# jay-tux/cutrace

Measured on AMD Instinct MI355X. Metric: Mrays/sec (primary+secondary), higher is better.
Workload: dtype f32; 1 GPU; bunny.json@1920x1080 bounces=5 fudge=1e-3, 1 frame(s)/step row-tiled over 1 GPU(s), gather to rank 0; steps_in_flight=1

## Files before the change

cutrace_amd/__init__.py:

```python
import contextlib
import ctypes as C
import os

import numpy as np

from . import _lib
from ._lib import Camera, Light, Material, Object, RenderStats, Rows, SceneDesc, Triangle, Vec3

ROOT = _lib.ROOT

VAR_AUTO = 0
VAR_NO_PREFILTER = 2
VAR_NO_ANYHIT = 4
VAR_NO_CLUSTER = 8
VAR_STATS = 16
VAR_EXACT_POW = 32
VAR_NO_REORDER = 256
VAR_NO_OCC6 = 512
VAR_NO_DIRECT = 1024
VAR_IMAGE_ORDER_FIRST = 2048
VAR_MERGE = 4096
VAR_IGNORE_TRANSPARENT = 8192

RAY_IGNORE_TRANSPARENT = 1
# ... 395 lines not shown
        shape = C.c_uint32()
        _check("ctr_debug_last_shape", _lib.hip_lib().ctr_debug_last_shape(self._h, C.byref(shape)))
        return int(shape.value)

    def last_opaque(self):
        opaque = C.c_uint32()
        _check("ctr_debug_last_opaque", _lib.hip_lib().ctr_debug_last_opaque(self._h, C.byref(opaque)))
        return int(opaque.value)

    def room_facts(self):
        out = np.zeros(5, np.float32)
        lights = C.c_uint32()
        _check("ctr_debug_room_facts", _lib.hip_lib().ctr_debug_room_facts(self._h, out.ctypes.data, C.byref(lights)))
        return {"c": out[:3].copy(), "r": float(out[3]), "delta": float(out[4]), "lights": int(lights.value)}

    @staticmethod
    def lane_stats(reset=True):
        raw = np.zeros(96, np.uint64)
        _check("ctr_debug_lane_stats", _lib.hip_lib().ctr_debug_lane_stats(raw.ctypes.data, 1 if reset else 0))
        c = [int(x) for x in raw]
        trips, live = c[72], c[73]
        out = {"wave_trips": trips, "live_lanes_per_trip": live / trips if trips else None,
               "live_fraction": live / (64.0 * trips) if trips else None,
               "live_fraction_of_in_image_lanes": (live / trips) / (c[75] / c[74]) if trips and c[74] and c[75] else None,
               "trips_by_live_lanes_1_8_to_57_64": c[64:72], "trips_mixing_kinds": c[76], "waves": c[74],
               "merged_walks": c[78], "merged_walks_redone": c[77],
               "shadow_casts_at_meshes": {"wave_casts": c[80], "receivers_all_off_mesh": c[81], "of_those_unoccluded_by_meshes": c[82],
                                          "unoccluded_by_meshes_any_receiver": c[83]},
               "anyhit_shadow_trips": c[88], "anyhit_shadow_trips_without_planes": c[89]}
        kinds = {}
        for d in range(16):
            for name, base in (("radiance", 0), ("shadow", 16)):
                if c[32 + base + d]:
                    label = "primary" if (name == "radiance" and d == 0) else f"{name}@depth{d}"
                    kinds[label] = {"lanes": c[base + d], "trips": c[32 + base + d],
                                    "lanes_per_trip": c[base + d] / c[32 + base + d]}
        out["by_kind"] = kinds
        return out

    def _torch_device(self):
        import torch
        return torch.device("cuda", self.device)

    def _rays_arg(self, x, what, cols):
# ... 453 lines not shown
```

cutrace_amd/_lib.py:

```python
import ctypes as C
import os

PKG = os.path.dirname(os.path.abspath(__file__))
ROOT = os.path.dirname(PKG)


class Vec3(C.Structure):
    _fields_ = [("x", C.c_float), ("y", C.c_float), ("z", C.c_float)]

    def tup(self):
        return (self.x, self.y, self.z)


class Triangle(C.Structure):
    _fields_ = [("p1", Vec3), ("p2", Vec3), ("p3", Vec3)]


class Object(C.Structure):
    _fields_ = [("type", C.c_uint32), ("reserved", C.c_uint32), ("mat_idx", C.c_uint64),
                ("v0", Vec3), ("v1", Vec3), ("v2", Vec3), ("f0", C.c_float),
                ("tri_begin", C.c_uint64), ("tri_count", C.c_uint64)]


class Light(C.Structure):
# ... 137 lines not shown
        "ctr_scene_set_cameras": ([_ptr, _P(Camera), _u32], _int),
        "ctr_render_device_batch": ([_ptr, _f32, _int, _P(Rows), _u32, _u32, _u64, _u32, _ptr, _ptr, _ptr, _ptr, _ptr], _int),
        "ctr_algorithmic_bytes": ([_ptr, _f32, _int, _P(Rows), _P(_u64), _P(_u64)], _int),
        "ctr_frame_alloc": ([_u64, _P(_f32p), _P(_f32p), _P(_f32p)], _int),
        "ctr_frame_free": ([_f32p], None),
        "ctr_tile_costs": ([_ptr, _ptr, _u64, _P(_u64)], _int),
        "ctr_last_counters": ([_ptr, _ptr], _int),
        "ctr_selftest_exact_math": ([_P(_u64)], _int),
        "ctr_debug_poison_next_order": ([_ptr], _int),
        "ctr_render_uv": ([_ptr, _f32, _int, _P(Rows), _ptr, _ptr, _ptr, _ptr, _P(RenderStats)], _int),
        "ctr_debug_lane_stats": ([_ptr, _int], _int),
        "ctr_debug_last_kernel": ([_ptr, _P(_u32)], _int),
        "ctr_debug_last_shape": ([_ptr, _P(_u32)], _int),
        "ctr_debug_last_opaque": ([_ptr, _P(_u32)], _int),
        "ctr_debug_room_facts": ([_ptr, _ptr, _P(_u32)], _int),
        "ctr_multi_create": ([_P(SceneDesc), _P(_int), _int, _P(_ptr)], _int),
        "ctr_multi_destroy": ([_ptr], None),
        "ctr_multi_devices": ([_ptr], _int),
        "ctr_multi_transport": ([_ptr], _str),
        "ctr_multi_size": ([_ptr, _P(_u64), _P(_u64)], _int),
        "ctr_multi_set_size": ([_ptr, _u64, _u64], _int),
        "ctr_multi_set_variant": ([_ptr, _u32], _int),
        "ctr_render_multi": ([_ptr, _f32, _int, _u64, _ptr, _ptr, _ptr, _P(RenderStats)], _int),
        "ctr_multi_kernel_ms": ([_ptr, _P(C.c_double), _int], _int),
        "ctr_reinterleave_device": ([_P(ReintPart), _u32, _u64, _u64, _u64, _ptr, _ptr, _ptr, _ptr], _int),
        "ctr_multi_submit": ([_ptr, _f32, _int, _u64, _ptr, _ptr, _ptr], _int),
        "ctr_multi_wait": ([_ptr, _P(RenderStats)], _int),
    },
    "cutrace_rays.h": {
        "ctr_cast_rays": ([_ptr, _P(RayQuery), _ptr], _int),
# ... 103 lines not shown
```

cutrace_amd/csrc/ctr_internal.h:

```cpp
#ifndef CUTRACE_AMD_CTR_INTERNAL_H
#define CUTRACE_AMD_CTR_INTERNAL_H

#include <hip/hip_runtime_api.h>
#include <string.h>

#include <memory>
#include <mutex>
#include <string>
#include <utility>
#include <vector>

#include "cutrace_amd.h"
#include "guard_scan.h"
#include "lbvh.h"
#include "mesh_refit.h"
#include "scene_device.h"
#include "scene_flatten.h"
#include "tile_order_policy.h"

#pragma GCC visibility push(hidden)
int fail(int code, const std::string &msg);
int hip_fail(hipError_t e, const char *what);
#define HIP_TRY(expr)                                     \
  do {                                                    \
// ... 51 lines not shown

struct ctr_scene {
  int device = 0;
  FlatScene flat;
  SceneBuf d_objs{sizeof(DObj)}, d_oloop{sizeof(DObj)}, d_meshes{sizeof(DObj)}, d_planes{sizeof(DPlanePair)}, d_tris{sizeof(DTri)};
  SceneBuf d_nodes{sizeof(DNode)}, d_nodes4{sizeof(DNode4)}, d_gnorm{4 * sizeof(float)}, d_lights{sizeof(DLight)}, d_mats{sizeof(DMat)};
  DCam cam{};
  GrowBuf d_cams{sizeof(DCam)};
  uint32_t n_cams = 0;
  uint32_t cams_epoch = 0;
  std::vector<DCam> h_cams;
  uint32_t user_variant = CTR_VAR_AUTO;
  bool no_scene_head = false;
  bool no_shape_build = false;
  bool no_wall_skip = false;
  bool no_opaque_build = false;
  struct RoomWords { float c[3], r, delta; uint32_t lights; } last_room{};
  GrowBuf out{7 * sizeof(float)};
  GrowBuf uv{2 * sizeof(float)};
  GrowBuf img{9};
  GrowBuf d_groups{sizeof(uint32_t)};
  GrowBuf h_groups{sizeof(uint32_t), true};
  GrowBuf h_counters{sizeof(unsigned long long), true};
  unsigned long long last_cnt[16] = {0};
  GrowBuf d_counters{sizeof(unsigned long long)};
  GrowBuf d_shards{sizeof(unsigned long long)};
  uint32_t last_kernel = 0;
  uint32_t last_shape = 0;
  uint32_t last_opaque = 0;
  OrderState order;
  GrowBuf d_cost{sizeof(uint32_t)}, d_order{sizeof(uint32_t)};
  bool poison_next_order = false;
// ... 56 lines not shown
```

cutrace_amd/csrc/ctr_render.cpp:

```cpp
#include <hip/hip_runtime_api.h>

#include <chrono>
#include <cstdio>
#include <cstdlib>

#include "ctr_internal.h"
#include "cutrace_aa.h"
#include "cutrace_images.h"
#include "cutrace_lens.h"
#include "frame_images.h"
#include "kernel_choice.h"
#include "row_parts.h"
#include "tile_order.h"
#include "tile_shape.h"

#ifndef CTR_OCC6_MIN_TRIS
#define CTR_OCC6_MIN_TRIS 1000
#endif

uint64_t ctr_scene::occ6_min_tris() {
  static const uint64_t v = [] { const char *e = getenv("CUTRACE_OCC6_MIN_TRIS"); return e ? (uint64_t)atoll(e) : (uint64_t)CTR_OCC6_MIN_TRIS; }();
  return v;
}

// ... 113 lines not shown
  L.h = s->cam.h;
  L.first_frame = c.first_frame;
  L.n_frames = c.n_frames;
  L.frame_stride_px = c.frame_stride_px;
  L.fudge = c.fudge;
  L.bounces = c.bounces;
  L.ss_log2 = c.ss_log2;
}

void set_root_and_head(const ctr_scene *s, RenderLaunch &L, bool merged) {
  if (merged) L.scene.tlas_root = BVH_LEAF_FLAG | s->flat.n_mesh;
  if (!s->no_scene_head) fill_scene_head(s->flat, L.scene.tlas_root, L.head);
  L.no_shape = s->no_shape_build ? 1u : 0u;
  L.no_opaque = s->no_opaque_build ? 1u : 0u;
  if ((L.variant & KV_ANYHIT) && (ctr_launch_shape(L) == KS_ONE_MESH || (L.variant & KV_STATS))) fill_room_facts(s->flat, L.head, s->no_wall_skip);
}

ctr_scene::RoomWords room_words(const RenderLaunch &L) {
  return {{L.head.room_c[0], L.head.room_c[1], L.head.room_c[2]}, L.head.room_r, L.head.room_delta, L.head.room_lights};
}

int prepare_outputs(ctr_scene *s, RenderLaunch &L, size_t spx, const HostFrame *z) {
  if (int st = s->h_counters.reserve(16)) return st;
  if (int st = s->out.reserve(spx)) return st;
  L.depth = s->out.as<float>();
  L.color = L.depth + spx;
  L.normal = L.depth + 4 * spx;
  if (!z) return CTR_OK;
  const size_t groups = (size_t)ctr_staging_groups(L);
  if (int st = reserve_both(s->d_groups, s->h_groups, groups)) return st;
// ... 118 lines not shown
  L.variant = choice.kv;
  if (c.lens) {
    L.ray_origin = c.lens->d_origin;
    L.ray_dir = c.lens->d_dir;
    L.ray_ambient = c.lens->ambient;
  }
  if (c.ss_log2 && (st = aa_scale(L.w, L.h, L.rows, c.ss_log2, err))) return fail(st, err);
  set_root_and_head(s, L, choice.merged);
  {
    std::lock_guard<std::mutex> lk(s->mtx);
    if ((st = attach_order(s, L, big_mesh(s), false))) return st;
    s->last_kernel = L.variant;
    s->last_shape = ctr_launch_shape(L);
    s->last_opaque = ctr_launch_opaque(L);
    s->last_room = room_words(L);
  }
  return launched(ctr_launch_render(L, c.stream), "render kernel launch");
}

int render_host(ctr_scene *s, const RenderCall &c) {
  auto t0 = std::chrono::high_resolution_clock::now();
  int st = check_args(s, c.bounces);
  if (st) return st;
  std::lock_guard<std::mutex> lk(s->mtx);
  HIP_TRY(hipSetDevice(s->device));
  RenderLaunch L{};
  fill_launch(s, c, L);
  std::string err;
  if ((st = make_rows(L.h, c.rows, L.rows, err))) return fail(st, err);
  const size_t px = (size_t)L.rows.n_rows * s->cam.w;
// ... 8 lines not shown
  }
  const bool direct = choice.direct;
  const size_t spx = direct ? (size_t)ctr_staging_pixels(L) : (px ? px : 1);
  if ((st = prepare_outputs(s, L, spx, direct ? &z : nullptr))) return st;
  L.counters = s->d_counters.as<unsigned long long>();
  if (choice.reject == KR_UV_STATS) return fail(CTR_E_INVALID, "ctr_render_uv / CTR_VAR_IGNORE_TRANSPARENT: not with the counting / statistics variants");
  L.variant = s->last_kernel = choice.kv;
  if (L.variant & KV_UV) {
    if ((st = s->uv.reserve(px))) return st;
    L.uv = s->uv.as<float>();
  }
  set_root_and_head(s, L, choice.merged);
  s->last_shape = ctr_launch_shape(L);
  s->last_opaque = ctr_launch_opaque(L);
  s->last_room = room_words(L);
  if ((st = attach_order(s, L, big_mesh(s), c.count))) return st;
  HIP_TRY(hipMemsetAsync(s->d_counters.p, 0, 16 * sizeof(unsigned long long), nullptr));
  HIP_TRY(hipEventRecord(s->ev0, nullptr));
  if ((st = launched(ctr_launch_render(L, nullptr), "render kernel launch"))) return st;
  HIP_TRY(hipEventRecord(s->ev1, nullptr));
  if (px && !direct && (st = c.images ? images_out(s, L, *c.images, px) : copy_out(s, L, c.out, px))) return st;
  HIP_TRY(hipMemcpyAsync(s->h_counters.p, s->d_counters.p, 16 * sizeof(unsigned long long), hipMemcpyDeviceToHost, nullptr));
  const size_t n_groups = direct ? (size_t)ctr_staging_groups(L) : 0;
  if (direct) HIP_TRY(hipMemcpyAsync(s->h_groups.p, s->d_groups.p, n_groups * sizeof(uint32_t), hipMemcpyDeviceToHost, nullptr));
  HIP_TRY(hipStreamSynchronize(nullptr));
  if (direct && (st = check_delivery(s, L, c.out, spx, n_groups))) return st;
  return report(s, L, t0, c);
}

}
// ... 109 lines not shown
```

cutrace_amd/csrc/ctr_scene.cpp:

```cpp
#include <hip/hip_runtime_api.h>

#include <cstdio>
#include <cstdlib>
#include <cstring>
#include <mutex>
#include <string>
#include <vector>

#include "ctr_internal.h"
#include "cutrace_amd.h"
#include "guard.h"
#include "scene_device.h"
#include "scene_flatten.h"

namespace {
thread_local std::string g_err;
}

int fail(int code, const std::string &msg) {
  g_err = msg;
  fprintf(stderr, "cutrace_amd: %s\n", msg.c_str());
  return code;
}
int hip_fail(hipError_t e, const char *what) {
// ... 231 lines not shown
  int ndev = 0;
  hipError_t e = hipGetDeviceCount(&ndev);
  if (e != hipSuccess || ndev <= 0) return fail(CTR_E_NO_DEVICE, "no HIP device available (and there is no CPU fallback)");
  if (device < 0 || device >= ndev) return fail(CTR_E_INVALID, "device index out of range");
  HIP_TRY(hipSetDevice(device));
  create_stamp("device check");

  FlatScene F;
  if (int st = flatten_scene(*d, F, err)) return fail(st, err);
  auto *s = new ctr_scene();
  s->device = device;
  s->cam = to_dcam(d->cam);
  s->no_scene_head = env_switch("CUTRACE_NO_SCENE_HEAD");
  s->no_shape_build = env_switch("CUTRACE_NO_SHAPE_BUILD");
  s->no_wall_skip = env_switch("CUTRACE_NO_WALL_SKIP");
  s->no_opaque_build = env_switch("CUTRACE_NO_OPAQUE_BUILD");

  if (int st = upload_scene(s, F)) {
    ctr_scene_destroy(s);
    return hip_fail((hipError_t)(st - CTR_E_HIP_BASE), "scene upload");
  }
  create_stamp("device allocation + upload");
  s->n_cams = 1;
  s->flat = std::move(F);
  s->h_cams.assign(1, s->cam);
  create_stamp("host copies");
  if (int st = refresh_linear_meshes(s)) {
    ctr_scene_destroy(s);
    return st;
  }
// ... 99 lines not shown
  std::lock_guard<std::mutex> lk(s->mtx);
  *opaque = s->last_opaque;
  return CTR_OK;
}

int ctr_debug_room_facts(ctr_scene *s, float *out5, uint32_t *lights) {
  if (!s || !out5 || !lights) return fail(CTR_E_INVALID, "ctr_debug_room_facts: null argument");
  std::lock_guard<std::mutex> lk(s->mtx);
  for (int q = 0; q < 3; q++) out5[q] = s->last_room.c[q];
  out5[3] = s->last_room.r;
  out5[4] = s->last_room.delta;
  *lights = s->last_room.lights;
  return CTR_OK;
}

int ctr_last_counters(ctr_scene *s, uint64_t *out16) {
  if (!s || !out16) return fail(CTR_E_INVALID, "ctr_last_counters: null argument");
  std::lock_guard<std::mutex> lk(s->mtx);
  for (int q = 0; q < 16; q++) out16[q] = s->last_cnt[q];
  return CTR_OK;
}

}
```

cutrace_amd/csrc/render_kernel.hip:

```cpp
#include <hip/hip_runtime.h>
#include <math.h>
#include <stddef.h>
#include <stdint.h>
#include <stdlib.h>

#include "cutrace_amd.h"
#include "scene_device.h"
#include "bvh.h"
#include "kernel_choice.h"
#include "tile_order.h"
#include "tile_shape.h"
#include "vec3.h"

#define CADDR __attribute__((address_space(4)))
#define BALLOT(p) __builtin_amdgcn_ballot_w64(p)
#define HIDE_UNIFORM(x) asm volatile("" : "+v"(x))
#define PIN3(a, b, c) asm volatile("" : "+v"(a), "+v"(b), "+v"(c))
#define INVB(m) __builtin_amdgcn_inverse_ballot_w64(m)
#define FCMP(a, b, pred) __builtin_amdgcn_fcmpf((a), (b), (pred))
enum { FC_OEQ = 1, FC_OGT = 2, FC_OGE = 3, FC_OLT = 4, FC_OLE = 5 };
#define TL_NONE 0x7FFFFFFFu

extern "C" __device__ uint32_t ctr_writelane(uint32_t value, uint32_t lane, uint32_t old) __asm("llvm.amdgcn.writelane.i32");

// ... 104 lines not shown
  n = s;
  float y = __builtin_amdgcn_rcpf(s);
  const float e = __builtin_fmaf(-s, y, 1.0f);
  y = __builtin_fmaf(e, y, y);
  float q = y;
  const float r0 = __builtin_fmaf(-s, q, 1.0f);
  q = __builtin_fmaf(r0, y, q);
  const float r1 = __builtin_fmaf(-s, q, 1.0f);
  inv = __builtin_fmaf(r1, y, q);
}
__device__ __forceinline__ V3 vnormalized_n(V3 a, float &n) {
  float inv;
  norm_and_inverse(a.x * a.x + a.y * a.y + a.z * a.z, n, inv);
  return vscale(a, inv);
}
enum { F_R = 0, F_G, F_B, F_MAT, F_PX, F_PY, F_PZ, F_DX, F_DY, F_DZ };

struct KArgs {
  const CADDR DPlanePair *planes;
  uint32_t n_plane_recs, n_axis_recs, n_oloop, n_mesh, tlas_root, has_mesh;
  const CADDR DObj *objs;
  const CADDR float *gnorm;
  const CADDR DLight *lights;
  const CADDR DMat *mats;
  uint32_t n_light;
  int bounces;
  uint32_t n_obj, tlas_root2;
  const CADDR DObj *oloop;
  const CADDR DObj *meshes;
  uint32_t tlas_begin;
// ... 22 lines not shown

static_assert(offsetof(KArgs, planes) == 0 && offsetof(KArgs, has_mesh) == 28, "KArgs: the hot block is the first eight dwords");
static_assert(offsetof(KArgs, objs) == 32 && offsetof(KArgs, mats) == 56 && offsetof(KArgs, bounces) == 68, "KArgs: the cold block follows");

struct KParams {
  KArgs A;
  float *depth_out, *color_out, *normal_out;
  unsigned long long *counters;
};
static_assert(offsetof(KArgs, ss_log2) == 288 && offsetof(KArgs, ray_origin) == 296 && offsetof(KArgs, head) == 320, "KArgs: the lens arguments lie in the padding behind ss_log2");
static_assert(sizeof(KArgs) % 64 == 0 && offsetof(KArgs, head) % 64 == 0 && offsetof(KParams, depth_out) == sizeof(KArgs), "KParams mirrors the kernel's parameter list; the scene head lies on 64-byte lines");


constexpr uint32_t MSP_SHADOW = 0x80000000u, MSP_DONE = 0x40000000u;
constexpr uint32_t MSP_ROOM = 0x20000000u;
#define MSP_ACTIVE(m) ((int)(m) < 0x40000000)
#define MSP_IS_SHADOW(m) ((int)(m) < 0)
#define MSP_IS_RADIANCE(m) ((uint32_t)(m) < 0x40000000u)
#define MSP_DEPTH(m) ((int)((m) & 0xFFFFu))
enum { ACT_NONE = 0, ACT_LIGHT = 1, ACT_BOUNCE = 2, ACT_UNWIND = 3 };

template <uint32_t KV, uint32_t SHAPE = KS_GENERAL, bool ROOM = false, uint32_t OPQ = KO_PARENT>
__global__ __launch_bounds__(WG_THREADS, (KV & KV_OCC6) ? 6 : CTR_MIN_WAVES_EU) void render_kernel(KArgs A, float *__restrict__ depth_out,
                                                            float *__restrict__ color_out,
                                                            float *__restrict__ normal_out,
                                                            unsigned long long *__restrict__ counters) {
  constexpr bool PREFILTER = (KV & KV_PREFILTER) != 0;
  constexpr bool ANYHIT = (KV & KV_ANYHIT) != 0;
  constexpr bool COUNT = (KV & KV_COUNT) != 0;
  constexpr bool BVH = (KV & KV_BVH) != 0;
#ifdef CTR_WAVELOG
  constexpr bool STATS = true;
#else
  constexpr bool STATS = (KV & KV_STATS) != 0;
#endif
  constexpr bool FASTPOW = (KV & KV_FASTPOW) != 0;
  constexpr bool HOSTOUT = (KV & KV_HOSTOUT) != 0;
// ... 1 lines not shown
  constexpr bool SS = (KV & KV_SS) != 0;
  static_assert(!SS || !((KV & (KV_HOSTOUT | KV_STATS | KV_UV)) != 0), "the supersampled frame leaves through device buffers, three outputs");
  constexpr bool IGNTR = (KV & KV_IGNTR) != 0;
  constexpr bool MERGE = (KV & KV_MERGE) != 0;
  static_assert(!MERGE || BVH, "the merged tree is a BVH walk");
  constexpr bool RAYS = (KV & KV_RAYS) != 0;
  static_assert(!RAYS || !((KV & (KV_HOSTOUT | KV_STATS | KV_UV | KV_COUNT | KV_IGNTR | KV_MERGE)) != 0), "the lens render leaves through device buffers, three outputs, two-level walk");
  constexpr bool ONE_MESH = SHAPE == KS_ONE_MESH;
  static_assert(SHAPE == KS_GENERAL || SHAPE == KS_ONE_MESH, "launch shapes: kernel_choice.h");
  static_assert(!ROOM || ONE_MESH, "room-safe lanes: the one-mesh builds");
  constexpr bool ROOM_CODE = ANYHIT && (ROOM || STATS);
  static_assert(!ONE_MESH || (KV & ~(KV_OCC6 | KV_HOSTOUT)) == (KV_PREFILTER | KV_BVH | KV_ANYHIT | KV_FASTPOW), "KS_ONE_MESH: the builds of CTR_SHAPE_KERNELS");
  constexpr bool OPAQUE = OPQ != KO_PARENT;
  static_assert(OPQ == KO_PARENT || OPQ == KO_OPAQUE, "opaque builds: kernel_choice.h");
  static_assert(!OPAQUE || (ANYHIT && ONE_MESH), "the opaque builds are any-hit one-mesh builds");
  unsigned long long st[11] = {0, 0, 0, 0, 0, 0, 0, 0, 0, 0, 0};
#ifdef CTR_TIMING
  unsigned long long tm[10] = {0, 0, 0, 0, 0, 0, 0, 0, 0, 0};
  const unsigned long long tm_start = __builtin_readcyclecounter();
#define TSTAMP(v) const unsigned long long v = __builtin_readcyclecounter()
#define TACC(i, a, b) tm[i] += (b) - (a)
#else
#define TSTAMP(v)
#define TACC(i, a, b)
#endif

#ifdef CTR_WAVELOG
  const unsigned long long wl_start = __builtin_amdgcn_s_memrealtime();
#endif
  CTR_MARK(0);
// ... 164 lines not shown
      }
      const mask_t img_m = BALLOT(in_image);
      if (lane == 0) {
        const uint32_t n_live = (uint32_t)__builtin_popcountll(active_m);
        atomicAdd(&g_lane_stats[64 + ((n_live - 1u) >> 3)], 1ull);
        atomicAdd(&g_lane_stats[72], 1ull);
        atomicAdd(&g_lane_stats[73], (unsigned long long)n_live);
        if (kinds > 1u) atomicAdd(&g_lane_stats[76], 1ull);
        if (first_trip) { atomicAdd(&g_lane_stats[74], 1ull); atomicAdd(&g_lane_stats[75], (unsigned long long)__builtin_popcountll(img_m)); }
      }
    }

    float best = INFINITY;
    int bobj = -1, btri = -1;
    mask_t alive_m = active_m;
    V3 rinv = mk(0, 0, 0);
    bool have_rinv = false;
    V3 ria = mk(0, 0, 0);
    float ria_big = 0.f;
    float cmax = 0.f;
    if (k_has_mesh) {
      CTR_MARK(2);
      ria = mk(fminf(fmaxf(__builtin_amdgcn_rcpf(rd.x), -1e30f), 1e30f),
               fminf(fmaxf(__builtin_amdgcn_rcpf(rd.y), -1e30f), 1e30f),
               fminf(fmaxf(__builtin_amdgcn_rcpf(rd.z), -1e30f), 1e30f));
      ria_big = fmaxf(fmaxf(fabsf(ria.x), fabsf(ria.y)), fabsf(ria.z));
      cmax = fmaxf(fmaxf(fabsf(rd.x), fabsf(rd.y)), fabsf(rd.z));
    }

    TSTAMP(t_loop0);
    TACC(0, t_trip0, t_loop0);
    CTR_MARK(3);
    const bool anyhit_cast = ANYHIT && shadow_cast;
    const bool ign_now = IGNTR && first_trip;
    bool skip_planes = false;
    if constexpr (ROOM_CODE) {
      if (hd_room_lights != 0u) {
        const mask_t safe_m = BALLOT((((hd_room_lights >> (li & 31u)) & (msp >> 29)) & 1u) != 0u);
        skip_planes = (alive_m & ~(shadow_m & safe_m)) == 0ull;
      }
      if (STATS && shadow_m != 0ull && lane == 0) {
        atomicAdd(&g_lane_stats[88], 1ull);
        atomicAdd(&g_lane_stats[89], skip_planes ? 1ull : 0ull);
      }
    }
    if (!skip_planes) {
      mask_t live_m = alive_m;
      const float mt_lo = min_t - fabsf(min_t) * 0x1p-21f;
      float lhv = anyhit_cast ? light_dist : best;
      lhv = lhv + fabsf(lhv) * 0x1p-21f;
      float tiny = 1e-37f;
      asm volatile("" : "+v"(tiny));
      auto plane_exact = [&](uint32_t pidx, float num, float den, mask_t need_m, auto site) -> bool {
        CTR_MARK(110 + decltype(site)::value);
        bool retire = false;
        if (INVB(need_m)) {
          const float t0 = num / den;
          if (__builtin_isfinite(t0) && t0 > min_t) {
            if (t0 < best || (t0 == best && (int)pidx < bobj)) {
              best = t0; bobj = (int)pidx; btri = -1;
// ... 305 lines not shown
              CTR_MARK(88);
              if (STATS && lane == 0) atomicAdd(&g_lane_stats[77], 1ull);
              t_pend = AK->tlas_root2;
              t_sp = 0u;
              continue;
            }
          } else bb_m = box_test(O, live_m, SITE(0));
          TSTAMP(t_bb);
          TACC(3, t_tl0, t_bb);
          CTR_MARK(21);
          if (bb_m == 0ull) continue;
          CTR_MARK(22);
          const uint32_t beg = o_tri_begin, cnt = o_tri_count;
          if (COUNT) n_aabb_tris += INVB(bb_m) ? (unsigned long long)cnt : 0ull;
          if (STATS) st[4]++;
          uint32_t pl_nodes = 0, pl_tris = 0;
          float mt = INFINITY;
          uint32_t morig = 0xFFFFFFFFu;
          const bool anyhit_now = ANYHIT && shadow_cast;
          const mask_t anyhit_m = ANYHIT ? shadow_m : 0ull;
          const bool t_filter = A.fudge >= 1e-30f;
          float lim = anyhit_now ? light_dist : best;

          const float2_ ro_xy = {ro.x, ro.y};
          auto tri_test = [&](const TriR &T, uint32_t tri_index, mask_t lanes_m) {
            CTR_MARK(23);
            mask_t c_m = lanes_m;
            if (STATS) { st[2]++; st[7] += __builtin_popcountll(lanes_m); pl_tris += INVB(lanes_m) ? 1u : 0u; }
            const float2_ dxy = T.pxy - ro_xy;
            const float dx = dxy.x, dy = dxy.y, dz = T.pz - ro.z;
// ... 470 lines not shown
            const float2_ ox = {ro.x, ro.x}, oy = {ro.y, ro.y}, oz = {ro.z, ro.z};
            const float2_ n0 = (pr(0) - ox) * pr(1), n1 = (pr(2) - oy) * pr(3), n2 = (pr(4) - oz) * pr(5);
            const float num_max = fmaxf(fmaxf(fmaxf(n0.x, n0.y), n1.x), fmaxf(fmaxf(n1.y, n2.x), n2.y));
            const float room_r = __uint_as_float(rm_rest[1]);
            const bool in_box = fabsf(ro.x - __uint_as_float(rm_c01[0])) <= room_r && fabsf(ro.y - __uint_as_float(rm_c01[1])) <= room_r &&
                                fabsf(ro.z - __uint_as_float(rm_rest[0])) <= room_r;
            msp |= (in_box && num_max <= __uint_as_float(rm_rest[2])) ? MSP_ROOM : 0u;
          }
        }
      }
    } else if (MSP_IS_SHADOW(msp)) {
      CTR_MARK(43);
      { const CADDR DLight &L1 = k_lights[li + 1u]; nl_type = L1.type; nl_v = mk(L1.vx, L1.vy, L1.vz); }
      bool done_shadow;
      float shadow_fac = 0.f;
      if (was_hit && best < light_dist) {
        const float trans = ANYHIT ? 0.0f : k_mats[k_objs[bobj].mat].transparency;
        if (!ANYHIT) intensity += (1.0f - trans);
        if (ANYHIT || intensity >= 1.0f) { shadow_fac = 1.0f; done_shadow = true; }
        else {
          min_t = (float)((double)best + 1e-3);
          done_shadow = false;
        }
      } else {
        shadow_fac = ANYHIT ? 0.0f : intensity;
        done_shadow = true;
      }
      if (done_shadow) {
        if (shadow_fac < 1.0f) {
          CTR_MARK(44);
          const CADDR DMat &M = k_mats[mat_i];
          const CADDR DLight &Lg = k_lights[li];
          const V3 diffuse = mk(M.cx, M.cy, M.cz);
          const V3 specular = vscale(diffuse, M.specular);
          const V3 color = mk(Lg.cx, Lg.cy, Lg.cz);
          const V3 nd = rd;
          const V3 nn_ = get_nn();
          const float fd = smax(0.0f, vdot(nn_, nd));
          const V3 ld = vmul(diffuse, color);
          const V3 hsum = vadd(vscale(get_in_dn(), -1.0f), nd);
          const V3 hv = FASTPOW ? vscale(hsum, __builtin_amdgcn_rsqf(vdot(hsum, hsum))) : vnormalized(hsum);
          const float sx = smax(0.0f, vdot(nn_, hv));
          float fs;
          if (FASTPOW) {
            fs = (M.phong_exp == 0.0f) ? 1.0f : __builtin_amdgcn_exp2f(M.phong_exp * __builtin_amdgcn_logf(sx));
          } else {
            fs = (float)pow((double)sx, (double)M.phong_exp);
          }
          const V3 ls = vmul(specular, color);
          fin = vadd(fin, vscale(vadd(vscale(ld, fd), vscale(ls, fs)), 1 - shadow_fac));
        }
        CTR_MARK(45);
        li++;
        act = ACT_LIGHT;
      }
    }

    TSTAMP(t_cont_mid);
    TACC(7, t_loop1, t_cont_mid);
    CTR_MARK(46);
    if (act == ACT_LIGHT) {
      if (li < k_n_light) {
// ... 6 lines not shown
          direction = vscale(lg_v, -1.0f);
          distance = INFINITY;
        } else {
          CTR_MARK(48);
          const V3 diff = vsub(lg_v, ro);
          direction = vnormalized_n(diff, distance);
          CTR_MARK(94);
        }
        CTR_MARK(49);
        float dir_norm;
        rd = vnormalized_n(direction, dir_norm);
        CTR_MARK(95);
        light_dist = distance * dir_norm;
        intensity = 0.0f;
        min_t = (float)(0.0 + 1e-3);
        msp |= MSP_SHADOW;
      } else {
        act = ACT_BOUNCE;
      }
    }

    if (act == ACT_BOUNCE) {
      CTR_MARK(50);
      const CADDR DMat &M = k_mats[mat_i];
      const float reflective = M.reflexivity, translucent = OPAQUE ? 0.0f : M.transparency;
      const int sp = MSP_DEPTH(msp);
      const bool more = sp < k_bounces;
      const bool do_refl = more && (double)reflective >= 1e-6;
      const bool do_trans = !OPAQUE && more && (double)translucent >= 1e-6;
      if (do_refl || do_trans) {
        CTR_MARK(51);
// ... 196 lines not shown
    if (lane == 0) {
      tm[9] = __builtin_readcyclecounter() - tm_start;
      for (int q = 0; q < 10; q++) atomicAdd(&sh[4 + q], tm[q]);
    }
#endif
    if (lane == 0) {
      atomicAdd(&sh[0], c);
      atomicMax(&sh[1], (unsigned long long)dbits);
      if (COUNT) atomicAdd(&sh[2], t);
    }
  }
}
#undef CTR_MARK

bool launch_head_mesh(const RenderLaunch &L) {
  return L.head.n_mesh == 1u && (L.scene.tlas_root & BVH_LEAF_FLAG) && L.scene.n_mesh != 0u;
}

int launch(const RenderLaunch &L, uint32_t kv, const void *kernel, hipStream_t stream) {
  KArgs A;
  const DScene &S = L.scene;
  A.objs = (const CADDR DObj *)S.objs;
  A.oloop = (const CADDR DObj *)S.oloop;
  A.meshes = (const CADDR DObj *)S.meshes;
  A.n_mesh = S.n_mesh;
  A.head = L.head;
  const bool head_mesh = launch_head_mesh(L);
  const bool head_axis = L.head.n_axis_recs == 3u && S.n_axis_recs >= 3u && S.n_plane_recs >= 3u;
  A.tlas_root = S.tlas_root | (head_mesh ? CTR_TL_HEAD_FLAG : 0u);
  A.tlas_root2 = S.tlas_root_regular;
  A.tlas_begin = S.tlas_begin;
// ... 134 lines not shown

uint32_t ctr_launch_opaque(const RenderLaunch &L) { return opaque_build(L.variant, ctr_launch_shape(L), L.no_opaque != 0u); }

int ctr_launch_render(const RenderLaunch &L, void *stream) {
  const void *kernel;
  switch (L.variant) {
#define X(kv) case (kv): kernel = (const void *)render_kernel<(kv)>; break;
    CTR_RENDER_KERNELS(X)
    CTR_LENS_KERNELS(X)
#undef X
    default: return (int)hipErrorInvalidValue;
  }
  if (ctr_launch_shape(L) == KS_ONE_MESH) {
    const uint32_t opq = ctr_launch_opaque(L);
    const bool room = L.head.room_lights != 0u;
    switch (L.variant) {
#define Y(kv, o) (room ? (const void *)render_kernel<(kv), KS_ONE_MESH, true, o> : (const void *)render_kernel<(kv), KS_ONE_MESH, false, o>)
#define X(kv) case (kv): kernel = opq == KO_OPAQUE ? Y(kv, KO_OPAQUE) : Y(kv, KO_PARENT); break;
      CTR_SHAPE_KERNELS(X)
#undef X
#undef Y
      default: return (int)hipErrorInvalidValue;
    }
  }
  return launch(L, L.variant, kernel, (hipStream_t)stream);
}
```

cutrace_amd/csrc/scene_device.h:

```cpp
#ifndef CUTRACE_AMD_SCENE_DEVICE_H
#define CUTRACE_AMD_SCENE_DEVICE_H

#include <stddef.h>
#include <stdint.h>

struct DTri {
  float ab[3][2];
  float px, py, pz;
  uint32_t orig;
  float nx, ny, nz;
  float ke;
  float ke2;
  float pad1;
};
static_assert(sizeof(DTri) == 64, "DTri must be one 64-byte line");

#define CTR_OBJ_MERGED 4u
#define CTR_MERGE_MAX_MESHES 255u
struct DObj {
  uint32_t type;
  uint32_t mat;
  uint32_t tri_begin;
  uint32_t tri_count;
  uint32_t node_begin;
// ... 53 lines not shown
struct DRows {
  uint32_t row_begin;
  uint32_t row_end;
  uint32_t part_stride;
  uint32_t n_rows;
  uint32_t block_rows;
  uint32_t part, n_parts;
  uint32_t first_block;
};

struct alignas(64) DSceneHead {
  float ax[6][2];
  uint32_t ax_index[6];
  uint32_t ax_transparent[6];
  uint32_t n_axis_recs;
  uint32_t n_mesh;
  float room_c[3], room_r;
  float room_delta;
  uint32_t room_lights;
  DObj mesh;
};
static_assert(sizeof(DSceneHead) == 192 && offsetof(DSceneHead, mesh) == 128 && offsetof(DSceneHead, room_c) == 104,
              "DSceneHead: two 64-byte lines of planes, one of mesh");
#define CTR_TL_HEAD_FLAG 0x40000000u

struct DScene {
  const DObj *objs;
  const DObj *oloop;
  const DObj *meshes;
  const DPlanePair *planes;
  const DTri *tris;
  const void *nodes;
  const void *nodes4;
  const float *gnorm;
  const DLight *lights;
  const DMat *mats;
  uint32_t n_mesh, tlas_root, tlas_begin;
  uint32_t tlas_root_regular;
// ... 48 lines not shown
```

cutrace_amd/csrc/scene_flatten.cpp:

```cpp
#include "scene_flatten.h"

#include <algorithm>
#include <atomic>
#include <chrono>
#include <cmath>
#include <cstdio>
#include <cstdlib>
#include <cstring>
#include <thread>

#include "tri_record.h"

namespace {

std::vector<BvhInput> tri_boxes(const ctr_triangle *src, size_t n) {
  std::vector<BvhInput> prims(n);
  for (size_t q = 0; q < n; q++) {
    const ctr_vec3 *v[3] = {&src[q].p1, &src[q].p2, &src[q].p3};
    BvhInput &b = prims[q];
    for (int a = 0; a < 3; a++) {
      const float c0 = (&v[0]->x)[a], c1 = (&v[1]->x)[a], c2 = (&v[2]->x)[a];
      b.mn[a] = fminf(c0, fminf(c1, c2));
      b.mx[a] = fmaxf(c0, fmaxf(c1, c2));
      b.c[a] = 0.5f * (b.mn[a] + b.mx[a]);
// ... 243 lines not shown
}

void shading_flags(FlatScene &F) {
  auto largest = [](float x, float y, float z) { return std::max(std::fabs((double)x), std::max(std::fabs((double)y), std::fabs((double)z))); };
  double lambda = 0.0, worst = 0.0;
  for (const DLight &l : F.lights) lambda += largest(l.cx, l.cy, l.cz);
  F.all_opaque = true;
  F.need_cold = F.any_bounce = false;
  for (const DMat &m : F.mats) {
    if (!(m.transparency == 0.0f)) F.all_opaque = false;
    if ((double)m.transparency >= 1e-6 && (double)m.reflexivity >= 1e-6) F.need_cold = true;
    if ((double)m.transparency >= 1e-6 || (double)m.reflexivity >= 1e-6) F.any_bounce = true;
    worst = std::max(worst, std::fabs((double)m.phong_exp * (double)m.specular) * largest(m.cx, m.cy, m.cz));
  }
  F.fast_pow_ok = fast_pow_in_bar(worst, lambda);
}

}

uint32_t ray_stack_slots(const FlatScene &F) {
  uint32_t deepest = 0;
  std::vector<std::pair<uint32_t, uint32_t>> todo;
  for (const MeshGuard &g : F.guards) {
    if (g.mesh_pos < 0 || g.node_count == 0) continue;
    todo.assign(1, {0u, 1u});
    while (!todo.empty()) {
      const auto [n, lvl] = todo.back();
      todo.pop_back();
      deepest = std::max(deepest, lvl);
      const DNode4 &N = F.nodes4[g.node_begin + n];
// ... 544 lines not shown
void fill_scene_head(const FlatScene &F, uint32_t tlas_root, DSceneHead &H) {
  H = DSceneHead{};
  if (F.n_axis_recs >= 3u && F.planes.size() >= 3u) {
    for (int r = 0; r < 3; r++)
      for (int k = 0; k < 2; k++) {
        H.ax[2 * r][k] = F.planes[r].p[r][k];
        H.ax[2 * r + 1][k] = F.planes[r].n[r][k];
        H.ax_index[2 * r + k] = F.planes[r].index[k];
        H.ax_transparent[2 * r + k] = F.planes[r].transparent[k];
      }
    H.n_axis_recs = 3u;
  }
  const uint32_t leaf = tlas_root & 0xFFFFFFu;
  if (F.n_mesh != 0u && (tlas_root & BVH_LEAF_FLAG) && leaf < F.meshes.size()) {
    H.mesh = F.meshes[leaf];
    H.n_mesh = 1u;
  }
}

void room_facts(DSceneHead &H, const DLight *lights, size_t n_light, const RoomTuning &tune) {
  for (int a = 0; a < 3; a++) H.room_c[a] = 0.0f;
  H.room_r = H.room_delta = 0.0f;
  H.room_lights = 0u;
  if (H.n_axis_recs != 3u || n_light == 0 || n_light > 32) return;
  struct Slot { int a; double p, n; };
  Slot slots[6];
  int n_slots = 0;
  double lo[3] = {INFINITY, INFINITY, INFINITY}, hi[3] = {-INFINITY, -INFINITY, -INFINITY};
  for (int k = 0; k < 6; k++) {
    if (H.ax_index[k] == CTR_PLANE_PAD) continue;
    const int a = k / 2;
// ... 41 lines not shown
      const double s_max = (std::fabs((double)c[S.a] - S.p) + r_eff) * std::fabs(S.n);
      ok = s_l > 0.0 && s_l >= tune.k * 0x1p-24 * (t_max * std::fabs(S.n) + s_max);
      den_i = std::min(den_i, s_l / t_max);
    }
    if (ok) { mask |= 1u << i; den_min = std::min(den_min, den_i); }
  }
  if (mask == 0u) return;
  const float delta = (float)(0.5 * (double)(float)1e-3 * den_min * (1.0 - 0x1p-20) * tune.delta_scale);
  if (!(delta >= 1e-30f) || !std::isfinite(delta)) return;
  for (int a = 0; a < 3; a++) H.room_c[a] = c[a];
  H.room_r = r;
  H.room_delta = delta;
  H.room_lights = mask;
}

void fill_room_facts(const FlatScene &F, DSceneHead &H, bool switched_off) {
  if (!switched_off && F.planes.size() == 3u && F.n_axis_recs == 3u && F.all_opaque) room_facts(H, F.lights.data(), F.lights.size());
  else room_facts(H, nullptr, 0);
}

bool env_switch(const char *name) {
  const char *e = getenv(name);
  return e && atoi(e) != 0;
}
```

cutrace_amd/csrc/scene_flatten.h:

```cpp
#ifndef CUTRACE_AMD_SCENE_FLATTEN_H
#define CUTRACE_AMD_SCENE_FLATTEN_H

#include <stdint.h>
#include <string>
#include <vector>

#include "bvh.h"
#include "cutrace_amd.h"
#include "scene_device.h"

#ifndef CTR_BVH_LEAF
#define CTR_BVH_LEAF 4
#endif
constexpr uint32_t BVH_LEAF = CTR_BVH_LEAF;

#define CTR_GUARD_SLOTS 64u
constexpr uint64_t CTR_MESH_TRIS_MAX = 0xFFFFFFull;
constexpr uint64_t CTR_SCENE_TRIS_MAX = 0x7FFFFFFFull;
#define CTR_MERGED_SPARE_NODES ((CTR_GUARD_SLOTS + 2u) / 3u)

struct MeshGuard {
  uint32_t node_begin = 0, node_count = 0;
  uint32_t node_cap = 0;
  uint32_t tri_begin = 0, tri_count = 0;
// ... 30 lines not shown
  std::vector<DPlanePair> planes;
  std::vector<DTri> tris;
  std::vector<DNode> nodes;
  std::vector<DNode4> nodes4;
  std::vector<float> gn;
  std::vector<DLight> lights;
  std::vector<DMat> mats;
  uint32_t n_mesh = 0, tlas_root = BVH_LEAF_FLAG, tlas_begin = 0;
  float tl_mn[3] = {0, 0, 0}, tl_mx[3] = {0, 0, 0};
  uint32_t n_axis_recs = 0;
  bool has_mesh = false;
  bool all_opaque = true;
  bool need_cold = false;
  bool any_bounce = false;
  bool fast_pow_ok = true;
  uint64_t mesh_tris = 0;
  size_t mesh_bytes = 0;
  std::vector<MeshGuard> guards;
  Merged merged;
  struct FreeRange { uint32_t begin, count; };
  std::vector<FreeRange> free_tris, free_nodes4;
  uint32_t ray_slots = 0;
};

constexpr double CTR_FAST_POW_KAPPA = 2.42e-7;
constexpr double CTR_COLOUR_TOL = 1e-4;
inline bool fast_pow_in_bar(double worst, double lambda) { return 2.0 * CTR_FAST_POW_KAPPA * worst * lambda <= CTR_COLOUR_TOL; }

int validate_desc(const ctr_scene_desc &d, std::string &err);
int flatten_scene(const ctr_scene_desc &d, FlatScene &F, std::string &err);
// ... 38 lines not shown
std::vector<DirtyRange> mesh_joined(FlatScene &F, size_t gi, const float *box);
std::vector<DirtyRange> object_removed(FlatScene &F, size_t i, long *guard_removed);
struct SceneRoom { uint64_t tris_live, tris_total, nodes4_live, nodes4_total; };
SceneRoom scene_room(const FlatScene &F);

__attribute__((visibility("hidden"))) void fill_scene_counts(const FlatScene &F, DScene &D);

void fill_scene_head(const FlatScene &F, uint32_t tlas_root, DSceneHead &H);

struct RoomTuning {
  double k = 16.0;
  double delta_scale = 1.0;
};
void room_facts(DSceneHead &H, const DLight *lights, size_t n_light, const RoomTuning &tune = RoomTuning());
void fill_room_facts(const FlatScene &F, DSceneHead &H, bool switched_off);
bool env_switch(const char *name);

DNode4 empty_node4();
inline void unbounded_box(DNode4 &N, int c) {
  for (int a = 0; a < 3; a++) { N.lo[a][c] = -3.0e38f; N.hi[a][c] = 3.0e38f; }
}

void create_stamp(const char *what);

#endif
```

include/cutrace_amd.h:

```cpp
#ifndef CUTRACE_AMD_H
#define CUTRACE_AMD_H

#include <stdint.h>

#ifdef __cplusplus
extern "C" {
#endif

#define CTR_ABI_VERSION 3

#define CTR_OK 0
#define CTR_E_INVALID 1
#define CTR_E_NO_DEVICE 2
#define CTR_E_IO 3
#define CTR_E_PARSE 4
#define CTR_E_DELIVERY 5
#define CTR_E_HIP_BASE 1000

typedef struct ctr_vec3 { float x, y, z; } ctr_vec3;

enum { CTR_OBJ_TRIANGLE = 0, CTR_OBJ_MESH = 1, CTR_OBJ_PLANE = 2, CTR_OBJ_SPHERE = 3 };
enum { CTR_LIGHT_SUN = 0, CTR_LIGHT_POINT = 1 };
enum { CTR_MAT_PHONG = 0 };

// ... 107 lines not shown
#define CTR_VAR_NO_DIRECT 1024u
#define CTR_VAR_MERGE 4096u
#define CTR_VAR_IGNORE_TRANSPARENT 8192u
#define CTR_VAR_NO_OCC6 512u
int ctr_set_variant(ctr_scene *scene, uint32_t variant_bits);
int ctr_selftest_exact_math(uint64_t *n_mismatch);
int ctr_last_counters(ctr_scene *scene, uint64_t *out16);
int ctr_debug_lane_stats(uint64_t *out96, int reset);
int ctr_render_uv(ctr_scene *scene, float fudge, int bounces, const ctr_rows *rows, float *depth, float *color3,
                  float *normal3, float *uv2, ctr_render_stats *stats);
int ctr_debug_poison_next_order(ctr_scene *scene);
int ctr_debug_last_kernel(ctr_scene *scene, uint32_t *kv);
int ctr_debug_last_shape(ctr_scene *scene, uint32_t *shape);
int ctr_debug_last_opaque(ctr_scene *scene, uint32_t *opaque);
int ctr_debug_room_facts(ctr_scene *scene, float *out5, uint32_t *lights);
int ctr_tile_costs(ctr_scene *scene, uint32_t *out, uint64_t capacity, uint64_t *n_tiles);

int ctr_algorithmic_bytes(ctr_scene *scene, float fudge, int bounces, const ctr_rows *rows,
                          uint64_t *bytes, uint64_t *ray_count);

#ifdef __cplusplus
}
#endif
#endif
```

Before: 79850 Mrays/s.

## Skip shadow ray traversal for lights whose shading contribution is exactly zero

Before casting a shadow ray, each lane checks whether the diffuse and specular terms for that light are both exactly zero. If they are, the lane is marked dark and drops out of BVH traversal, and a wave made entirely of dark lanes skips the mesh and plane walks. The skip is enabled only for opaque one-mesh scenes whose material and light colours are finite and bounded, so that skipping cannot change the result. In exchange it adds per-shadow-ray shading math, ballots and another kernel template specialisation.

```diff
diff --git a/cutrace_amd/__init__.py b/cutrace_amd/__init__.py
--- a/cutrace_amd/__init__.py
+++ b/cutrace_amd/__init__.py
@@ -433,6 +433,11 @@
         _check("ctr_debug_room_facts", _lib.hip_lib().ctr_debug_room_facts(self._h, out.ctypes.data, C.byref(lights)))
         return {"c": out[:3].copy(), "r": float(out[3]), "delta": float(out[4]), "lights": int(lights.value)}
 
+    def dark_skip(self):
+        word = C.c_uint32()
+        _check("ctr_debug_dark_skip", _lib.hip_lib().ctr_debug_dark_skip(self._h, C.byref(word)))
+        return int(word.value)
+
     @staticmethod
     def lane_stats(reset=True):
         raw = np.zeros(96, np.uint64)
@@ -446,7 +451,8 @@
                "merged_walks": c[78], "merged_walks_redone": c[77],
                "shadow_casts_at_meshes": {"wave_casts": c[80], "receivers_all_off_mesh": c[81], "of_those_unoccluded_by_meshes": c[82],
                                           "unoccluded_by_meshes_any_receiver": c[83]},
-               "anyhit_shadow_trips": c[88], "anyhit_shadow_trips_without_planes": c[89]}
+               "anyhit_shadow_trips": c[88], "anyhit_shadow_trips_without_planes": c[89],
+               "dark_lights": {"lane_light_pairs": c[90], "shadow_trips_all_dark": c[91], "mesh_entries_with_a_dark_lane": c[92]}}
         kinds = {}
         for d in range(16):
             for name, base in (("radiance", 0), ("shadow", 16)):
diff --git a/cutrace_amd/_lib.py b/cutrace_amd/_lib.py
--- a/cutrace_amd/_lib.py
+++ b/cutrace_amd/_lib.py
@@ -175,6 +175,7 @@
         "ctr_debug_last_shape": ([_ptr, _P(_u32)], _int),
         "ctr_debug_last_opaque": ([_ptr, _P(_u32)], _int),
         "ctr_debug_room_facts": ([_ptr, _ptr, _P(_u32)], _int),
+        "ctr_debug_dark_skip": ([_ptr, _P(_u32)], _int),
         "ctr_multi_create": ([_P(SceneDesc), _P(_int), _int, _P(_ptr)], _int),
         "ctr_multi_destroy": ([_ptr], None),
         "ctr_multi_devices": ([_ptr], _int),
diff --git a/cutrace_amd/csrc/ctr_internal.h b/cutrace_amd/csrc/ctr_internal.h
--- a/cutrace_amd/csrc/ctr_internal.h
+++ b/cutrace_amd/csrc/ctr_internal.h
@@ -89,8 +89,10 @@
   bool no_scene_head = false;
   bool no_shape_build = false;
   bool no_wall_skip = false;
+  bool no_dark_skip = false;
   bool no_opaque_build = false;
   struct RoomWords { float c[3], r, delta; uint32_t lights; } last_room{};
+  uint32_t last_dark_skip = 0;
   GrowBuf out{7 * sizeof(float)};
   GrowBuf uv{2 * sizeof(float)};
   GrowBuf img{9};
diff --git a/cutrace_amd/csrc/ctr_render.cpp b/cutrace_amd/csrc/ctr_render.cpp
--- a/cutrace_amd/csrc/ctr_render.cpp
+++ b/cutrace_amd/csrc/ctr_render.cpp
@@ -151,6 +151,7 @@
   L.no_shape = s->no_shape_build ? 1u : 0u;
   L.no_opaque = s->no_opaque_build ? 1u : 0u;
   if ((L.variant & KV_ANYHIT) && (ctr_launch_shape(L) == KS_ONE_MESH || (L.variant & KV_STATS))) fill_room_facts(s->flat, L.head, s->no_wall_skip);
+  if ((L.variant & KV_ANYHIT) && (ctr_launch_opaque(L) == KO_OPAQUE || (L.variant & KV_STATS))) fill_dark_skip(s->flat, L.head, s->no_dark_skip);
 }
 
 ctr_scene::RoomWords room_words(const RenderLaunch &L) {
@@ -299,6 +300,7 @@
     s->last_shape = ctr_launch_shape(L);
     s->last_opaque = ctr_launch_opaque(L);
     s->last_room = room_words(L);
+    s->last_dark_skip = (L.head.mesh_dark & CTR_HEAD_DARK) ? 1u : 0u;
   }
   return launched(ctr_launch_render(L, c.stream), "render kernel launch");
 }
@@ -337,6 +339,7 @@
   s->last_shape = ctr_launch_shape(L);
   s->last_opaque = ctr_launch_opaque(L);
   s->last_room = room_words(L);
+  s->last_dark_skip = (L.head.mesh_dark & CTR_HEAD_DARK) ? 1u : 0u;
   if ((st = attach_order(s, L, big_mesh(s), c.count))) return st;
   HIP_TRY(hipMemsetAsync(s->d_counters.p, 0, 16 * sizeof(unsigned long long), nullptr));
   HIP_TRY(hipEventRecord(s->ev0, nullptr));
diff --git a/cutrace_amd/csrc/ctr_scene.cpp b/cutrace_amd/csrc/ctr_scene.cpp
--- a/cutrace_amd/csrc/ctr_scene.cpp
+++ b/cutrace_amd/csrc/ctr_scene.cpp
@@ -269,6 +269,7 @@
   s->no_scene_head = env_switch("CUTRACE_NO_SCENE_HEAD");
   s->no_shape_build = env_switch("CUTRACE_NO_SHAPE_BUILD");
   s->no_wall_skip = env_switch("CUTRACE_NO_WALL_SKIP");
+  s->no_dark_skip = env_switch("CUTRACE_NO_DARK_SKIP");
   s->no_opaque_build = env_switch("CUTRACE_NO_OPAQUE_BUILD");
 
   if (int st = upload_scene(s, F)) {
@@ -398,6 +399,13 @@
   return CTR_OK;
 }
 
+int ctr_debug_dark_skip(ctr_scene *s, uint32_t *word) {
+  if (!s || !word) return fail(CTR_E_INVALID, "ctr_debug_dark_skip: null argument");
+  std::lock_guard<std::mutex> lk(s->mtx);
+  *word = s->last_dark_skip;
+  return CTR_OK;
+}
+
 int ctr_last_counters(ctr_scene *s, uint64_t *out16) {
   if (!s || !out16) return fail(CTR_E_INVALID, "ctr_last_counters: null argument");
   std::lock_guard<std::mutex> lk(s->mtx);
diff --git a/cutrace_amd/csrc/render_kernel.hip b/cutrace_amd/csrc/render_kernel.hip
--- a/cutrace_amd/csrc/render_kernel.hip
+++ b/cutrace_amd/csrc/render_kernel.hip
@@ -142,6 +142,17 @@
   norm_and_inverse(a.x * a.x + a.y * a.y + a.z * a.z, n, inv);
   return vscale(a, inv);
 }
+__device__ __forceinline__ float light_fd(V3 nn_, V3 nd) { return smax(0.0f, vdot(nn_, nd)); }
+template <bool FAST>
+__device__ __forceinline__ float light_fs(V3 nn_, V3 in_dn_, V3 nd, const CADDR DMat &M) {
+  const V3 hsum = vadd(vscale(in_dn_, -1.0f), nd);
+  const V3 hv = FAST ? vscale(hsum, __builtin_amdgcn_rsqf(vdot(hsum, hsum))) : vnormalized(hsum);
+  const float sx = smax(0.0f, vdot(nn_, hv));
+  float fs;
+  if (FAST) fs = (M.phong_exp == 0.0f) ? 1.0f : __builtin_amdgcn_exp2f(M.phong_exp * __builtin_amdgcn_logf(sx));
+  else fs = (float)pow((double)sx, (double)M.phong_exp);
+  return fs;
+}
 enum { F_R = 0, F_G, F_B, F_MAT, F_PX, F_PY, F_PZ, F_DX, F_DY, F_DZ };
 
 struct KArgs {
@@ -194,13 +205,14 @@
 
 constexpr uint32_t MSP_SHADOW = 0x80000000u, MSP_DONE = 0x40000000u;
 constexpr uint32_t MSP_ROOM = 0x20000000u;
+constexpr uint32_t MSP_DARK = 0x10000000u;
 #define MSP_ACTIVE(m) ((int)(m) < 0x40000000)
 #define MSP_IS_SHADOW(m) ((int)(m) < 0)
 #define MSP_IS_RADIANCE(m) ((uint32_t)(m) < 0x40000000u)
 #define MSP_DEPTH(m) ((int)((m) & 0xFFFFu))
 enum { ACT_NONE = 0, ACT_LIGHT = 1, ACT_BOUNCE = 2, ACT_UNWIND = 3 };
 
-template <uint32_t KV, uint32_t SHAPE = KS_GENERAL, bool ROOM = false, uint32_t OPQ = KO_PARENT>
+template <uint32_t KV, uint32_t SHAPE = KS_GENERAL, bool ROOM = false, uint32_t OPQ = KO_PARENT, bool DARK = false>
 __global__ __launch_bounds__(WG_THREADS, (KV & KV_OCC6) ? 6 : CTR_MIN_WAVES_EU) void render_kernel(KArgs A, float *__restrict__ depth_out,
                                                             float *__restrict__ color_out,
                                                             float *__restrict__ normal_out,
@@ -232,6 +244,8 @@
   constexpr bool OPAQUE = OPQ != KO_PARENT;
   static_assert(OPQ == KO_PARENT || OPQ == KO_OPAQUE, "opaque builds: kernel_choice.h");
   static_assert(!OPAQUE || (ANYHIT && ONE_MESH), "the opaque builds are any-hit one-mesh builds");
+  static_assert(!DARK || OPAQUE, "dark lights: the opaque builds");
+  constexpr bool DARK_CODE = DARK || (ANYHIT && STATS);
   unsigned long long st[11] = {0, 0, 0, 0, 0, 0, 0, 0, 0, 0, 0};
 #ifdef CTR_TIMING
   unsigned long long tm[10] = {0, 0, 0, 0, 0, 0, 0, 0, 0, 0};
@@ -426,12 +440,17 @@
     float best = INFINITY;
     int bobj = -1, btri = -1;
     mask_t alive_m = active_m;
+    mask_t dark_m = 0ull;
+    if constexpr (DARK_CODE) dark_m = BALLOT((msp & MSP_DARK) != 0u);
+    if constexpr (DARK) alive_m &= ~dark_m;
+    const bool all_dark = DARK && alive_m == 0ull;
+    if (DARK_CODE && STATS && shadow_m != 0ull && (active_m & ~dark_m) == 0ull && lane == 0) atomicAdd(&g_lane_stats[91], 1ull);
     V3 rinv = mk(0, 0, 0);
     bool have_rinv = false;
     V3 ria = mk(0, 0, 0);
     float ria_big = 0.f;
     float cmax = 0.f;
-    if (k_has_mesh) {
+    if (k_has_mesh && !all_dark) {
       CTR_MARK(2);
       ria = mk(fminf(fmaxf(__builtin_amdgcn_rcpf(rd.x), -1e30f), 1e30f),
                fminf(fmaxf(__builtin_amdgcn_rcpf(rd.y), -1e30f), 1e30f),
@@ -456,6 +475,7 @@
         atomicAdd(&g_lane_stats[89], skip_planes ? 1ull : 0ull);
       }
     }
+    if constexpr (DARK) skip_planes = skip_planes || all_dark;
     if (!skip_planes) {
       mask_t live_m = alive_m;
       const float mt_lo = min_t - fabsf(min_t) * 0x1p-21f;
@@ -791,6 +811,7 @@
           const uint32_t beg = o_tri_begin, cnt = o_tri_count;
           if (COUNT) n_aabb_tris += INVB(bb_m) ? (unsigned long long)cnt : 0ull;
           if (STATS) st[4]++;
+          if (DARK_CODE && STATS && dark_m != 0ull && lane == 0) atomicAdd(&g_lane_stats[92], 1ull);
           uint32_t pl_nodes = 0, pl_tris = 0;
           float mt = INFINITY;
           uint32_t morig = 0xFFFFFFFFu;
@@ -1291,7 +1312,8 @@
       { const CADDR DLight &L1 = k_lights[li + 1u]; nl_type = L1.type; nl_v = mk(L1.vx, L1.vy, L1.vz); }
       bool done_shadow;
       float shadow_fac = 0.f;
-      if (was_hit && best < light_dist) {
+      const bool dark_lane = DARK && (msp & MSP_DARK) != 0u;
+      if ((was_hit && best < light_dist) || dark_lane) {
         const float trans = ANYHIT ? 0.0f : k_mats[k_objs[bobj].mat].transparency;
         if (!ANYHIT) intensity += (1.0f - trans);
         if (ANYHIT || intensity >= 1.0f) { shadow_fac = 1.0f; done_shadow = true; }
@@ -1313,16 +1335,21 @@
           const V3 color = mk(Lg.cx, Lg.cy, Lg.cz);
           const V3 nd = rd;
           const V3 nn_ = get_nn();
-          const float fd = smax(0.0f, vdot(nn_, nd));
+          float fd, fs;
           const V3 ld = vmul(diffuse, color);
-          const V3 hsum = vadd(vscale(get_in_dn(), -1.0f), nd);
-          const V3 hv = FASTPOW ? vscale(hsum, __builtin_amdgcn_rsqf(vdot(hsum, hsum))) : vnormalized(hsum);
-          const float sx = smax(0.0f, vdot(nn_, hv));
-          float fs;
-          if (FASTPOW) {
-            fs = (M.phong_exp == 0.0f) ? 1.0f : __builtin_amdgcn_exp2f(M.phong_exp * __builtin_amdgcn_logf(sx));
+          if constexpr (DARK_CODE) {
+            fd = light_fd(nn_, nd);
+            fs = light_fs<FASTPOW>(nn_, get_in_dn(), nd, M);
           } else {
-            fs = (float)pow((double)sx, (double)M.phong_exp);
+            fd = smax(0.0f, vdot(nn_, nd));
+            const V3 hsum = vadd(vscale(get_in_dn(), -1.0f), nd);
+            const V3 hv = FASTPOW ? vscale(hsum, __builtin_amdgcn_rsqf(vdot(hsum, hsum))) : vnormalized(hsum);
+            const float sx = smax(0.0f, vdot(nn_, hv));
+            if (FASTPOW) {
+              fs = (M.phong_exp == 0.0f) ? 1.0f : __builtin_amdgcn_exp2f(M.phong_exp * __builtin_amdgcn_logf(sx));
+            } else {
+              fs = (float)pow((double)sx, (double)M.phong_exp);
+            }
           }
           const V3 ls = vmul(specular, color);
           fin = vadd(fin, vscale(vadd(vscale(ld, fd), vscale(ls, fs)), 1 - shadow_fac));
@@ -1359,7 +1386,35 @@
         light_dist = distance * dir_norm;
         intensity = 0.0f;
         min_t = (float)(0.0 + 1e-3);
-        msp |= MSP_SHADOW;
+        if constexpr (DARK_CODE) {
+          uint32_t hd_dark = 1u;
+          if constexpr (!DARK) {
+            const CADDR KArgs *AD = AK;
+            asm volatile("" : "+s"(AD));
+            hd_dark = AD->head.mesh_dark & CTR_HEAD_DARK;
+          }
+          bool dark = false;
+          if (hd_dark != 0u) {
+            CTR_MARK(121);
+            const V3 nn_ = get_nn();
+            const bool fd_zero = (__float_as_uint(light_fd(nn_, rd)) & 0x7FFFFFFFu) == 0u;
+            if (BALLOT(fd_zero) != 0ull) {
+              CTR_MARK(122);
+              if (fd_zero) {
+                const float fs = light_fs<FASTPOW>(nn_, get_in_dn(), rd, k_mats[mat_i]);
+                dark = (__float_as_uint(fs) & 0x7FFFFFFFu) == 0u && __float_as_uint(fin.x) != 0x80000000u &&
+                       __float_as_uint(fin.y) != 0x80000000u && __float_as_uint(fin.z) != 0x80000000u;
+              }
+              if (STATS) {
+                const mask_t dk_m = BALLOT(dark);
+                if (dk_m != 0ull && lane_now() == (uint32_t)__builtin_ctzll(dk_m)) atomicAdd(&g_lane_stats[90], (unsigned long long)__builtin_popcountll(dk_m));
+              }
+            }
+          }
+          msp = (msp & ~MSP_DARK) | MSP_SHADOW | (dark ? MSP_DARK : 0u);
+        } else {
+          msp |= MSP_SHADOW;
+        }
       } else {
         act = ACT_BOUNCE;
       }
@@ -1586,7 +1641,7 @@
 #undef CTR_MARK
 
 bool launch_head_mesh(const RenderLaunch &L) {
-  return L.head.n_mesh == 1u && (L.scene.tlas_root & BVH_LEAF_FLAG) && L.scene.n_mesh != 0u;
+  return (L.head.mesh_dark & CTR_HEAD_MESH) != 0u && (L.scene.tlas_root & BVH_LEAF_FLAG) && L.scene.n_mesh != 0u;
 }
 
 int launch(const RenderLaunch &L, uint32_t kv, const void *kernel, hipStream_t stream) {
@@ -1751,9 +1806,10 @@
   if (ctr_launch_shape(L) == KS_ONE_MESH) {
     const uint32_t opq = ctr_launch_opaque(L);
     const bool room = L.head.room_lights != 0u;
+    const bool dark = opq == KO_OPAQUE && (L.head.mesh_dark & CTR_HEAD_DARK) != 0u;
     switch (L.variant) {
-#define Y(kv, o) (room ? (const void *)render_kernel<(kv), KS_ONE_MESH, true, o> : (const void *)render_kernel<(kv), KS_ONE_MESH, false, o>)
-#define X(kv) case (kv): kernel = opq == KO_OPAQUE ? Y(kv, KO_OPAQUE) : Y(kv, KO_PARENT); break;
+#define Y(kv, o, d) (room ? (const void *)render_kernel<(kv), KS_ONE_MESH, true, o, d> : (const void *)render_kernel<(kv), KS_ONE_MESH, false, o, d>)
+#define X(kv) case (kv): kernel = opq == KO_OPAQUE ? (dark ? Y(kv, KO_OPAQUE, true) : Y(kv, KO_OPAQUE, false)) : Y(kv, KO_PARENT, false); break;
       CTR_SHAPE_KERNELS(X)
 #undef X
 #undef Y
diff --git a/cutrace_amd/csrc/scene_device.h b/cutrace_amd/csrc/scene_device.h
--- a/cutrace_amd/csrc/scene_device.h
+++ b/cutrace_amd/csrc/scene_device.h
@@ -91,14 +91,16 @@
   uint32_t ax_index[6];
   uint32_t ax_transparent[6];
   uint32_t n_axis_recs;
-  uint32_t n_mesh;
+  uint32_t mesh_dark;
   float room_c[3], room_r;
   float room_delta;
   uint32_t room_lights;
   DObj mesh;
 };
-static_assert(sizeof(DSceneHead) == 192 && offsetof(DSceneHead, mesh) == 128 && offsetof(DSceneHead, room_c) == 104,
+static_assert(sizeof(DSceneHead) == 192 && offsetof(DSceneHead, mesh) == 128 && offsetof(DSceneHead, room_c) == 104 && offsetof(DSceneHead, mesh_dark) == 100,
               "DSceneHead: two 64-byte lines of planes, one of mesh");
+#define CTR_HEAD_MESH 1u
+#define CTR_HEAD_DARK 0x10000u
 #define CTR_TL_HEAD_FLAG 0x40000000u
 
 struct DScene {
diff --git a/cutrace_amd/csrc/scene_flatten.cpp b/cutrace_amd/csrc/scene_flatten.cpp
--- a/cutrace_amd/csrc/scene_flatten.cpp
+++ b/cutrace_amd/csrc/scene_flatten.cpp
@@ -281,6 +281,9 @@
     worst = std::max(worst, std::fabs((double)m.phong_exp * (double)m.specular) * largest(m.cx, m.cy, m.cz));
   }
   F.fast_pow_ok = fast_pow_in_bar(worst, lambda);
+  const uint32_t facts = shade_facts(F.mats.data(), F.mats.size(), F.lights.data(), F.lights.size());
+  F.shade_finite = (facts & 1u) != 0u;
+  F.shade_bounded = (facts & 2u) != 0u;
 }
 
 }
@@ -855,7 +858,7 @@
   const uint32_t leaf = tlas_root & 0xFFFFFFu;
   if (F.n_mesh != 0u && (tlas_root & BVH_LEAF_FLAG) && leaf < F.meshes.size()) {
     H.mesh = F.meshes[leaf];
-    H.n_mesh = 1u;
+    H.mesh_dark |= CTR_HEAD_MESH;
   }
 }
 
@@ -927,6 +930,22 @@
   H.room_lights = mask;
 }
 
+uint32_t shade_facts(const DMat *mats, size_t n_mat, const DLight *lights, size_t n_light) {
+  bool finite = true, bounded = true;
+  auto look = [&](float v) {
+    if (!std::isfinite(v)) finite = false;
+    if (!(std::fabs(v) <= CTR_SHADE_BOUND)) bounded = false;
+  };
+  for (size_t i = 0; i < n_mat; i++) { look(mats[i].cx); look(mats[i].cy); look(mats[i].cz); look(mats[i].specular); }
+  for (size_t i = 0; i < n_light; i++) { look(lights[i].cx); look(lights[i].cy); look(lights[i].cz); }
+  return (finite ? 1u : 0u) | (bounded ? 2u : 0u);
+}
+
+void fill_dark_skip(const FlatScene &F, DSceneHead &H, bool switched_off) {
+  const bool holds = !switched_off && F.shade_finite && F.shade_bounded && F.all_opaque;
+  H.mesh_dark = (H.mesh_dark & ~CTR_HEAD_DARK) | (holds ? CTR_HEAD_DARK : 0u);
+}
+
 void fill_room_facts(const FlatScene &F, DSceneHead &H, bool switched_off) {
   if (!switched_off && F.planes.size() == 3u && F.n_axis_recs == 3u && F.all_opaque) room_facts(H, F.lights.data(), F.lights.size());
   else room_facts(H, nullptr, 0);
diff --git a/cutrace_amd/csrc/scene_flatten.h b/cutrace_amd/csrc/scene_flatten.h
--- a/cutrace_amd/csrc/scene_flatten.h
+++ b/cutrace_amd/csrc/scene_flatten.h
@@ -68,6 +68,7 @@
   bool need_cold = false;
   bool any_bounce = false;
   bool fast_pow_ok = true;
+  bool shade_finite = true, shade_bounded = true;
   uint64_t mesh_tris = 0;
   size_t mesh_bytes = 0;
   std::vector<MeshGuard> guards;
@@ -136,6 +137,9 @@
 };
 void room_facts(DSceneHead &H, const DLight *lights, size_t n_light, const RoomTuning &tune = RoomTuning());
 void fill_room_facts(const FlatScene &F, DSceneHead &H, bool switched_off);
+#define CTR_SHADE_BOUND 0x1p40f
+uint32_t shade_facts(const DMat *mats, size_t n_mat, const DLight *lights, size_t n_light);
+void fill_dark_skip(const FlatScene &F, DSceneHead &H, bool switched_off);
 bool env_switch(const char *name);
 
 DNode4 empty_node4();
diff --git a/include/cutrace_amd.h b/include/cutrace_amd.h
--- a/include/cutrace_amd.h
+++ b/include/cutrace_amd.h
@@ -145,6 +145,7 @@
 int ctr_debug_last_shape(ctr_scene *scene, uint32_t *shape);
 int ctr_debug_last_opaque(ctr_scene *scene, uint32_t *opaque);
 int ctr_debug_room_facts(ctr_scene *scene, float *out5, uint32_t *lights);
+int ctr_debug_dark_skip(ctr_scene *scene, uint32_t *word);
 int ctr_tile_costs(ctr_scene *scene, uint32_t *out, uint64_t capacity, uint64_t *n_tiles);
 
 int ctr_algorithmic_bytes(ctr_scene *scene, float fudge, int bounces, const ctr_rows *rows,
```

Result: faster. 84040 Mrays/s, median of 6 (+5.2%).
